# dangeross/rust-bitcoinconsensus

Measured on AMD Instinct MI355X. Metric: ECDSA verifies/sec (node) at 1/2/4/8 MI355X; % of int-ALU roofline, higher is better.
Workload: dtype u32; 1 GPU; C2: synthetic P2WPKH inputs, BIP143 sighash + ECDSA verify (BASELINE.json configs[1]); inputs_per_gpu=1000000, global_inputs=1000000, parallelism=shard x1 (independent tuples, no collective)

## Files before the change

### rust-bitcoinconsensus_amd/csrc/pipeline.h

```cpp
#pragma once
#include <cstddef>
#include <cstdint>
#include <algorithm>
#include <cstring>
#include <vector>
#include <functional>

namespace bcc {

void* pinned_alloc(size_t bytes);
void pinned_free(void* p, size_t bytes) noexcept;
void pinned_trim();
template <class T>
struct PinnedAlloc {
    using value_type = T;
    PinnedAlloc() = default;
    template <class U>
    PinnedAlloc(const PinnedAlloc<U>&) {}
    T* allocate(size_t n) { return static_cast<T*>(pinned_alloc(n * sizeof(T))); }
    void deallocate(T* p, size_t n) noexcept { pinned_free(p, n * sizeof(T)); }
    template <class U>
    bool operator==(const PinnedAlloc<U>&) const { return true; }
    template <class U>
    bool operator!=(const PinnedAlloc<U>&) const { return false; }
// ... 392 lines not shown
    void pre_upload(unsigned t, const TupleRows& rows);
    int stage_der(const DerTuples& t);
    int run(void* stream, const LateMsgFill* late = nullptr);
    int run_sighash(void* stream);
    int run_ecdsa(void* stream);
    int fetch_verdicts(uint8_t* out);
    int fetch_msgs(uint8_t* out);
    size_t n_tuples() const { return n_rows_; }
    size_t n_key_hashes() const { return n_hash_; }
    size_t n_pre() const { return n_pre_ + n_tjob_ + n_wjob_; }
    size_t n_wtx() const { return n_wtx_; }
    size_t sighash_bytes() const { return sighash_bytes_; }
    size_t n_aux() const { return n_aux_; }
    size_t pre_blocks() const { return pre_blocks_ + tjob_blocks_; }
    size_t aux_blocks() const { return aux_blocks_; }
    int device() const { return dev_; }
    uint8_t *d_tag = nullptr, *d_x = nullptr, *d_y = nullptr, *d_r = nullptr, *d_s = nullptr,
            *d_m = nullptr, *d_v = nullptr;

private:
    int sync();
    void* pick(void* stream);
    int launch_front(struct ihipStream_t* st);
    int upload_on(struct ihipStream_t* rows_stream, struct ihipStream_t* rest_stream, int part = 3);
    bool up_pending_ = false;
    struct UpCopy {
        size_t dst;
        const void* src;
        size_t len;
        bool rows;
    };
    std::vector<UpCopy> up_copies_;
    bool up_msg_one_ = false;
    static constexpr unsigned PRE_MAX_SHARDS = 64;
    std::vector<uint8_t*> pre_buf_;
    size_t pre_cap_ = 0;
    std::vector<size_t> pre_rows_;
    unsigned pre_P_ = 0;
    bool pre_armed_ = false;
    void* pre_stream_ = nullptr;
    void* ev_pre_ = nullptr;
    bool gather_pending_ = false;
    std::vector<size_t> gather_row0_;
    int launch_after_front(struct ihipStream_t* st);
    int launch_key_hash(struct ihipStream_t* st);
    int run_stages(void* stream, const LateMsgFill* late);
    int put_late(struct ihipStream_t* st, const LateMsgFill* late);
    std::vector<uint32_t> late_rows_;
    std::vector<uint8_t> late_digs_;
    void* late_host_ = nullptr;
    uint8_t* late_dev_ = nullptr;
    size_t late_cap_ = 0;
    bool kh_done_ = false;
    int dev_;
    void* own_stream_ = nullptr;
    void* last_stream_ = nullptr;
    void* side_stream_ = nullptr;
    void* ev_fork_ = nullptr;
    void* ev_join_ = nullptr;
    void* ev_up_ = nullptr;
    void* ev_rows_up_ = nullptr;
    void* ev_block_ = nullptr;
    int wait(void* stream);
    SigScratch scratch_;
    void* arena_ = nullptr;
    size_t cap_ = 0;
    void* host_image_ = nullptr;
    size_t host_cap_ = 0;
    void* vbuf_ = nullptr;
    size_t vcap_ = 0;
    void* vbuf_dev_ = nullptr;
    bool v_queued_ = false;
    int ensure_vbuf();
    int queue_verdicts(struct ihipStream_t* st);
    size_t n_rows_ = 0, n_pre_ = 0, n_aux_ = 0, n_patch_ = 0, pre_blocks_ = 0, aux_blocks_ = 0;
    uint8_t *d_aux_ = nullptr, *d_pre_ = nullptr, *d_auxd_ = nullptr;
    uint32_t *d_aux_off_ = nullptr, *d_aux_nblk_ = nullptr, *d_pre_off_ = nullptr,
             *d_pre_nblk_ = nullptr, *d_pre_row_ = nullptr;
    PatchRec* d_patch_ = nullptr;
    size_t n_tjob_ = 0, tjob_blocks_ = 0;
    uint8_t *d_tpl_ = nullptr, *d_code_ = nullptr;
    TplJob* d_tjob_ = nullptr;
    size_t n_wtx_ = 0, n_wjob_ = 0, n_win_ = 0, sighash_bytes_ = 0;
    uint8_t *d_txraw_ = nullptr, *d_txd_ = nullptr, *d_zeros_ = nullptr;
    WtxRec* d_wtx_ = nullptr;
    WinJob* d_wjob_ = nullptr;
    uint32_t* d_intab_ = nullptr;
    size_t n_hash_ = 0;
    uint32_t* d_hrow_ = nullptr;
    uint8_t* d_hprog_ = nullptr;
    uint32_t* d_emap_ = nullptr;
    uint32_t* d_mmap_ = nullptr;
    size_t n_der_ = 0;
    const uint8_t *d_pub_ = nullptr, *d_sig_ = nullptr;
    const uint64_t *d_pub_off_ = nullptr, *d_sig_off_ = nullptr;
    uint64_t pub_base_ = 0, pub_bytes_ = 0, sig_base_ = 0, sig_bytes_ = 0;

public:
    int early_launch(const TupleRows* const* rows, size_t P, const SighashJobs* const* jobs = nullptr);
    void early_reset();
    size_t early_rows() const { return early_n_; }

private:
    void* early_stream_ = nullptr;
    void* ev_early_ = nullptr;
    bool early_pending_ = false;
    size_t early_n_ = 0;
    SigScratch early_scratch_;
    void* early_arena_ = nullptr;
    size_t early_cap_ = 0;
    void* early_host_ = nullptr;
    size_t early_host_cap_ = 0;
    void* early_sig_stream_ = nullptr;
    void* ev_early_up_ = nullptr;
    void* ev_early_sig_ = nullptr;
    bool early_msgs_ = false;
    uint8_t* early_msg_ = nullptr;
};

int gpu_early_launch(int device, const TupleRows* const* rows, size_t P,
                     const SighashJobs* const* jobs = nullptr);
void gpu_early_reset(int device);

void set_stage_threads(unsigned n);

void set_direct_upload(bool on);
bool direct_upload();

void release_device_thread_state();
void release_tuple_thread_state();

int tuple_thread_buffers(int device, size_t dbytes, size_t hbytes, void** dbuf, void** hbuf,
                         void** stream);
int comb_device_tables(int* dev, const uint32_t** gcomb, int* cus);

int gpu_verify_batch(int device, const SighashJobs& jobs, const TupleRows& rows, uint8_t* verdict,
                     double* stage_seconds = nullptr);
struct StagedRound;
StagedRound* gpu_staged_new(int device);
void gpu_staged_free(StagedRound* s);
int gpu_staged_stage(StagedRound* s, const SighashJobs* const* jobs, const TupleRows* const* rows,
                     size_t parts, double* stage_seconds);
int gpu_staged_pre_arm(StagedRound* s, unsigned P, size_t cap_rows);
void gpu_staged_pre_upload(StagedRound* s, unsigned t, const TupleRows& rows);
int gpu_staged_stage_der(StagedRound* s, const DerTuples& t, double* stage_seconds);
int gpu_verify_der(int device, const DerTuples& t, uint8_t* verdict);
int gpu_staged_run(StagedRound* s, uint8_t* verdict, const LateMsgFill* late);
int gpu_staged_launch(StagedRound* s, const LateMsgFill* late);
int gpu_staged_finish(StagedRound* s, uint8_t* verdict);

int gpu_verify_parts(int device, const SighashJobs* const* jobs, const TupleRows* const* rows,
                     size_t parts, uint8_t* verdict, double* stage_seconds = nullptr,
                     const LateMsgFill* late = nullptr);

}
```

### rust-bitcoinconsensus_amd/csrc/sighash.hip

```cpp
#include <atomic>
#include <chrono>
#include <cstdlib>
#include <memory>
#include <mutex>
#include <new>
#include <thread>
#include <vector>
#include <cstring>
#include <cstdio>

#include "gpu_common.h"
#include "pipeline.h"
#include "sha256_device.h"
#include "host/hashes.h"
#include "host/team.h"

namespace bcc {

__device__ __forceinline__ uint32_t bswap_u32(uint32_t x) { return __builtin_bswap32(x); }

struct ShaMid {
    uint32_t s[8];
};

template <bool kDouble, bool kMid>
__device__ __forceinline__ void sha256_msg_lane(const uint8_t* __restrict__ buf,
                                                const uint32_t* __restrict__ off_blk,
                                                const uint32_t* __restrict__ nblk, uint32_t m,
                                                uint8_t* __restrict__ out,
                                                const uint32_t* __restrict__ out_row,
                                                const ShaMid& mid) {
    const uint4* p = reinterpret_cast<const uint4*>(buf + (size_t)off_blk[m] * 64);
    uint32_t st[8];
    if (kMid) {
#pragma unroll
        for (int k = 0; k < 8; k++) st[k] = mid.s[k];
    } else {
        sha256_init_state(st);
    }
    const uint32_t nb = nblk[m];
    uint4 nxt[4];
#pragma unroll
    for (int q = 0; q < 4; q++) nxt[q] = p[q];
    for (uint32_t b = 0; b < nb; b++) {
        uint32_t w[16];
#pragma unroll
        for (int q = 0; q < 4; q++) {
            w[4 * q + 0] = bswap_u32(nxt[q].x);
            w[4 * q + 1] = bswap_u32(nxt[q].y);
            w[4 * q + 2] = bswap_u32(nxt[q].z);
            w[4 * q + 3] = bswap_u32(nxt[q].w);
        }
        if (b + 1 < nb) {
#pragma unroll
            for (int q = 0; q < 4; q++) nxt[q] = p[(b + 1) * 4 + q];
        }
        sha256_compress(st, w);
    }
    uint32_t d[8];
    if (kDouble) {
        sha256_of_digest(d, st);
    } else {
#pragma unroll
        for (int k = 0; k < 8; k++) d[k] = st[k];
    }
    uint32_t row = out_row ? out_row[m] : m;
    uint4* o = reinterpret_cast<uint4*>(out + (size_t)row * 32);
    o[0] = make_uint4(bswap_u32(d[0]), bswap_u32(d[1]), bswap_u32(d[2]), bswap_u32(d[3]));
    o[1] = make_uint4(bswap_u32(d[4]), bswap_u32(d[5]), bswap_u32(d[6]), bswap_u32(d[7]));
}

__device__ __forceinline__ void sha256d_msg_lane(const uint8_t* __restrict__ buf,
                                                 const uint32_t* __restrict__ off_blk,
                                                 const uint32_t* __restrict__ nblk, uint32_t m,
                                                 uint8_t* __restrict__ out,
                                                 const uint32_t* __restrict__ out_row) {
    sha256_msg_lane<true, false>(buf, off_blk, nblk, m, out, out_row, ShaMid{});
}

__global__ __launch_bounds__(256) void sha256d_msgs_kernel(const uint8_t* __restrict__ buf,
                                                           const uint32_t* __restrict__ off_blk,
                                                           const uint32_t* __restrict__ nblk,
                                                           uint32_t nmsg, uint8_t* __restrict__ out,
                                                           const uint32_t* __restrict__ out_row) {
    uint32_t m = blockIdx.x * blockDim.x + threadIdx.x;
    if (m < nmsg) sha256d_msg_lane(buf, off_blk, nblk, m, out, out_row);
}

__global__ __launch_bounds__(64) void sha256_aux_kernel(const uint8_t* __restrict__ buf,
                                                        const uint32_t* __restrict__ off_blk,
                                                        const uint32_t* __restrict__ nblk,
                                                        uint32_t n, uint8_t* __restrict__ out) {
    uint32_t m = blockIdx.x * blockDim.x + threadIdx.x;
    if (m < n) sha256_msg_lane<false, false>(buf, off_blk, nblk, m, out, nullptr, ShaMid{});
}

// ... 124 lines not shown
        tpl_words(g, 64 * b, nxt, w);
        if (b + 1 < fast_blocks) tpl_fetch(m, g, 64 * (b + 1), nxt);
        sha256_compress(st, w);
    }
    const uint32_t nblk = tpl_nblk(j);
    for (uint32_t b = fast_blocks; b < nblk; b++) {
        uint32_t w[16];
#pragma unroll
        for (int k = 0; k < 16; k++) w[k] = tpl_word(m, 64 * b + 4 * k);
        sha256_compress(st, w);
    }
    uint32_t d[8];
    sha256_of_digest(d, st);
    uint4* o = reinterpret_cast<uint4*>(out + (size_t)j.row * 32);
    o[0] = make_uint4(bswap_u32(d[0]), bswap_u32(d[1]), bswap_u32(d[2]), bswap_u32(d[3]));
    o[1] = make_uint4(bswap_u32(d[4]), bswap_u32(d[5]), bswap_u32(d[6]), bswap_u32(d[7]));
}

constexpr int XS_SLOT = 100;
constexpr int XS_WG = 64;

__device__ __noinline__ void xs_compress(uint8_t* slot) {
    const uint32_t* b = reinterpret_cast<const uint32_t*>(slot);
    uint32_t* st = reinterpret_cast<uint32_t*>(slot + 64);
    uint32_t w[16], s8[8];
#pragma unroll
    for (int k = 0; k < 16; k++) w[k] = bswap_u32(b[k]);
#pragma unroll
    for (int k = 0; k < 8; k++) s8[k] = st[k];
    sha256_compress(s8, w);
#pragma unroll
    for (int k = 0; k < 8; k++) st[k] = s8[k];
}

struct XSha {
    uint8_t* slot;
    uint32_t fill;
    uint32_t total;
};

__device__ __forceinline__ void xs_init(XSha& h, uint8_t* slot) {
    h.slot = slot;
    h.fill = 0;
    h.total = 0;
    uint32_t* st = reinterpret_cast<uint32_t*>(slot + 64);
    uint32_t iv[8];
    sha256_init_state(iv);
#pragma unroll
    for (int k = 0; k < 8; k++) st[k] = iv[k];
}

__device__ __forceinline__ void xs_put(XSha& h, const uint8_t* __restrict__ src, uint32_t n) {
    h.total += n;
    while (n) {
        const uint32_t take = min(n, 64u - h.fill);
        const uintptr_t a = reinterpret_cast<uintptr_t>(src);
        const uint32_t* w = reinterpret_cast<const uint32_t*>(a & ~(uintptr_t)3);
        const uint32_t sh = (uint32_t)(a & 3), nd = (sh + take + 3) >> 2;
        uint32_t v[17];
#pragma unroll
        for (int k = 0; k < 17; k++) v[k] = (uint32_t)k < nd ? w[k] : 0u;
        uint32_t r[16];
#pragma unroll
        for (int k = 0; k < 16; k++) r[k] = __builtin_amdgcn_alignbyte(v[k + 1], v[k], sh);
        uint8_t* dst = h.slot + h.fill;
        if ((h.fill & 3) == 0) {
            uint32_t* d4 = reinterpret_cast<uint32_t*>(dst);
#pragma unroll
            for (int k = 0; k < 16; k++)
                if ((uint32_t)(4 * k) < take) d4[k] = r[k];
        } else {
#pragma unroll
            for (int i = 0; i < 64; i++)
                if ((uint32_t)i < take) dst[i] = (uint8_t)(r[i >> 2] >> (8 * (i & 3)));
        }
        h.fill += take;
        src += take;
        n -= take;
        if (h.fill == 64) {
            xs_compress(h.slot);
            h.fill = 0;
        }
    }
}

__device__ __forceinline__ void xs_final_d(XSha& h, uint8_t* __restrict__ out) {
    const uint64_t bits = (uint64_t)h.total * 8;
    h.slot[h.fill++] = 0x80;
    if (h.fill > 56) {
        while (h.fill < 64) h.slot[h.fill++] = 0;
        xs_compress(h.slot);
        h.fill = 0;
    }
    while (h.fill < 56) h.slot[h.fill++] = 0;
#pragma unroll
    for (int k = 0; k < 8; k++) h.slot[56 + k] = (uint8_t)(bits >> (8 * (7 - k)));
    xs_compress(h.slot);
    const uint32_t* st = reinterpret_cast<const uint32_t*>(h.slot + 64);
    uint32_t d[8], e[8];
#pragma unroll
    for (int k = 0; k < 8; k++) d[k] = st[k];
    sha256_of_digest(e, d);
    uint4* o = reinterpret_cast<uint4*>(out);
    o[0] = make_uint4(bswap_u32(e[0]), bswap_u32(e[1]), bswap_u32(e[2]), bswap_u32(e[3]));
    o[1] = make_uint4(bswap_u32(e[4]), bswap_u32(e[5]), bswap_u32(e[6]), bswap_u32(e[7]));
}

constexpr int XW_BYTES = 128;
struct XWin {
    uint8_t* w;
    const uint32_t* t4;
    uint32_t base;
    uint32_t nd;
};

__device__ __noinline__ void xw_refill(uint8_t* w, const uint32_t* __restrict__ t4, uint32_t nd,
                                       uint32_t base) {
    const uint32_t d0 = base >> 2;
    uint32_t v[XW_BYTES / 4];
#pragma unroll
    for (int k = 0; k < XW_BYTES / 4; k++) v[k] = d0 + k < nd ? t4[d0 + k] : 0u;
    uint32_t* w4 = reinterpret_cast<uint32_t*>(w);
#pragma unroll
    for (int k = 0; k < XW_BYTES / 4; k++) w4[k] = v[k];
}

__device__ __forceinline__ uint32_t xw_byte(XWin& x, uint32_t pos) {
    if (pos - x.base >= (uint32_t)XW_BYTES) {
        x.base = pos & ~3u;
        xw_refill(x.w, x.t4, x.nd, x.base);
    }
    return x.w[pos - x.base];
}

__device__ __forceinline__ uint32_t wire_cs(XWin& x, uint32_t& pos) {
    const uint32_t c = xw_byte(x, pos++);
    if (c < 253) return c;
    uint32_t v = xw_byte(x, pos) | xw_byte(x, pos + 1) << 8;
    if (c == 253) {
        pos += 2;
        return v;
    }
    v |= xw_byte(x, pos + 2) << 16 | xw_byte(x, pos + 3) << 24;
    pos += c == 254 ? 4 : 8;
    return v;
}

__device__ __forceinline__ uint32_t be_word_at(const uint32_t* __restrict__ t4, uint32_t off) {
    const uint32_t q = off >> 2;
    return bswap_u32(__builtin_amdgcn_alignbyte(t4[q + 1], t4[q], off & 3));
}

template <class W>
__device__ __forceinline__ void sha256d_words(W word, uint32_t L, uint8_t* __restrict__ out) {
    uint32_t st[8];
    sha256_init_state(st);
    const uint32_t nb = (L + 8) / 64 + 1, full = L >> 2, rem = L & 3;
    for (uint32_t b = 0; b < nb; b++) {
        uint32_t w[16];
#pragma unroll
        for (int q = 0; q < 16; q++) {
            const uint32_t m = 16 * b + q;
            uint32_t v;
            if (m < full) {
                v = word(m);
            } else if (m == full) {
                const uint32_t d = rem ? word(m) : 0u;
                const uint32_t keep = rem ? 0xFFFFFFFFu << (32 - 8 * rem) : 0u;
                v = (d & keep) | (0x80u << (24 - 8 * rem));
            } else {
                v = 0u;
            }
            if (b + 1 == nb && q == 14) v = (uint32_t)((uint64_t)L >> 29);
            if (b + 1 == nb && q == 15) v = L << 3;
            w[q] = v;
        }
        sha256_compress(st, w);
    }
    uint32_t d[8];
    sha256_of_digest(d, st);
    uint4* o = reinterpret_cast<uint4*>(out);
    o[0] = make_uint4(bswap_u32(d[0]), bswap_u32(d[1]), bswap_u32(d[2]), bswap_u32(d[3]));
    o[1] = make_uint4(bswap_u32(d[4]), bswap_u32(d[5]), bswap_u32(d[6]), bswap_u32(d[7]));
}

__device__ __forceinline__ uint32_t wire_input(XWin& x, uint32_t& pos, uint32_t* seq) {
    const uint32_t po = pos;
    pos += 36;
// ... 45 lines not shown
                p0 = p1;
                p1 = p2;
                p2 = next();
                kf++;
            }
            uint32_t w[16];
#pragma unroll
            for (int q = 0; q < 16; q++) {
                const uint32_t m = 16 * b + q, k = m / 9;
                uint32_t v = 0u;
                if (m < L / 4) {
                    const uint32_t kk = k - kf;
                    const uint32_t po = kk == 0 ? p0 : kk == 1 ? p1 : p2;
                    v = be_word_at(t4, po + 4 * (m - 9 * k));
                } else if (m == L / 4) {
                    v = 0x80000000u;
                }
                if (b + 1 == nb && q == 14) v = L >> 29;
                if (b + 1 == nb && q == 15) v = L << 3;
                w[q] = v;
            }
            sha256_compress(st, w);
        }
        while (np < nin) next();
    } else if (role == 1) {
        const uint32_t L = 4 * nin, nb = (L + 8) / 64 + 1;
        for (uint32_t b = 0; b < nb; b++) {
            uint32_t w[16];
#pragma unroll
            for (int q = 0; q < 16; q++) {
                const uint32_t m = 16 * b + q;
                uint32_t v = 0u;
                if (m < nin) {
                    uint32_t sq;
                    wire_input(x, pos, &sq);
                    v = be_word_at(t4, sq);
                } else if (m == nin) {
                    v = 0x80000000u;
                }
                if (b + 1 == nb && q == 14) v = L >> 29;
                if (b + 1 == nb && q == 15) v = L << 3;
                w[q] = v;
            }
            sha256_compress(st, w);
        }
    } else {
        for (uint32_t k = 0; k < nin; k++) {
            uint32_t sq;
            wire_input(x, pos, &sq);
        }
        const uint32_t nout = wire_cs(x, pos), o0 = pos;
        for (uint32_t k = 0; k < nout && pos < r.tx_len; k++) {
            pos += 8;
            pos += wire_cs(x, pos);
        }
        const uint32_t o1 = min(pos, r.tx_len);
        sha256d_words([&](uint32_t m) { return be_word_at(t4, o0 + 4 * m); }, o1 - o0, d + 64);
        return;
    }
    uint32_t dd[8];
    sha256_of_digest(dd, st);
    uint4* o = reinterpret_cast<uint4*>(d + 32 * role);
    o[0] = make_uint4(bswap_u32(dd[0]), bswap_u32(dd[1]), bswap_u32(dd[2]), bswap_u32(dd[3]));
    o[1] = make_uint4(bswap_u32(dd[4]), bswap_u32(dd[5]), bswap_u32(dd[6]), bswap_u32(dd[7]));
}

__global__ __launch_bounds__(XS_WG) void sighash_front_kernel(
    const uint8_t* __restrict__ txraw, const WtxRec* __restrict__ recs, uint32_t nwtx,
    uint32_t* __restrict__ intab, uint8_t* __restrict__ txd, const uint8_t* __restrict__ tpl,
    const uint8_t* __restrict__ code, const TplJob* __restrict__ tjobs, uint32_t ntpl,
    const uint8_t* __restrict__ aux, const uint32_t* __restrict__ aux_off,
    const uint32_t* __restrict__ aux_nblk, uint32_t naux, uint8_t* __restrict__ auxd,
    uint8_t* __restrict__ msg) {
    __shared__ __attribute__((aligned(16))) uint8_t lds[XS_WG * (XW_BYTES + 4)];
    const uint32_t g = blockIdx.x * blockDim.x + threadIdx.x, nw = 3 * nwtx;
    if (g < nw)
        bip143_tx_lane(txraw, recs, nwtx, g, intab, txd, lds + threadIdx.x * (XW_BYTES + 4));
    else if (g - nw < ntpl)
        sha256d_tpl_lane(tpl, code, tjobs, g - nw, msg);
    else if (g - nw - ntpl < naux)
        sha256d_msg_lane(aux, aux_off, aux_nblk, g - nw - ntpl, auxd, nullptr);
}

__global__ __launch_bounds__(XS_WG) void bip143_in_kernel(const uint8_t* __restrict__ txraw,
                                                          const WtxRec* __restrict__ recs,
                                                          const WinJob* __restrict__ jobs,
                                                          uint32_t n, const uint32_t* __restrict__ intab,
                                                          const uint8_t* __restrict__ txd,
                                                          const uint8_t* __restrict__ code,
                                                          const uint8_t* __restrict__ zeros,
                                                          uint8_t* __restrict__ msg) {
    __shared__ __attribute__((aligned(16))) uint8_t lds[XS_WG * XS_SLOT];
    const uint32_t i = blockIdx.x * blockDim.x + threadIdx.x;
    if (i >= n) return;
    const WinJob* jp = jobs + i;
    const WinJob j = *jp;
    const WtxRec r = recs[j.tx];
    const uint8_t* t = txraw + r.tx_off;
    const uint8_t* d = txd + 96 * (size_t)j.tx;
    const uint32_t* tab = intab + 2 * ((size_t)r.in_base + j.nin);
    const bool acp = (j.hashtype & 0x80) != 0, none = (j.hashtype & 0x1f) == 2;
    XSha h;
    xs_init(h, lds + threadIdx.x * XS_SLOT);
    xs_put(h, t, 4);
    xs_put(h, acp ? zeros : d, 32);
    xs_put(h, acp || none ? zeros : d + 32, 32);
    xs_put(h, t + tab[0], 36);
    xs_put(h, code + j.code_off, j.code_len);
    xs_put(h, reinterpret_cast<const uint8_t*>(&jp->amount_lo), 8);
    xs_put(h, t + tab[1], 4);
    xs_put(h, none ? zeros : d + 64, 32);
    xs_put(h, t + r.tx_len - 4, 4);
    xs_put(h, reinterpret_cast<const uint8_t*>(&jp->hashtype), 4);
    xs_final_d(h, msg + 32 * (size_t)j.row);
}


__device__ __forceinline__ void xs_final_s(XSha& h, uint8_t* __restrict__ out) {
    const uint64_t bits = (uint64_t)h.total * 8;
    h.slot[h.fill++] = 0x80;
    if (h.fill > 56) {
        while (h.fill < 64) h.slot[h.fill++] = 0;
        xs_compress(h.slot);
        h.fill = 0;
    }
    while (h.fill < 56) h.slot[h.fill++] = 0;
#pragma unroll
    for (int k = 0; k < 8; k++) h.slot[56 + k] = (uint8_t)(bits >> (8 * (7 - k)));
    xs_compress(h.slot);
    const uint32_t* st = reinterpret_cast<const uint32_t*>(h.slot + 64);
    uint32_t* o = reinterpret_cast<uint32_t*>(out);
#pragma unroll
    for (int k = 0; k < 8; k++) o[k] = bswap_u32(st[k]);
}

__device__ __forceinline__ void xs_put_le(XSha& h, uint32_t v, uint32_t n) {
    h.total += n;
    for (uint32_t k = 0; k < n; k++) {
        h.slot[h.fill++] = (uint8_t)(v >> (8 * k));
        if (h.fill == 64) {
            xs_compress(h.slot);
            h.fill = 0;
        }
    }
}

__device__ __forceinline__ uint32_t wire_txout(XWin& x, uint32_t& pos) {
    const uint32_t p0 = pos;
    pos += 8;
    pos += wire_cs(x, pos);
    return pos - p0;
}

__global__ __launch_bounds__(XS_WG) void taproot_tx_kernel(const uint8_t* __restrict__ raw,
                                                           const TtxRec* __restrict__ recs,
                                                           uint32_t n, uint32_t* __restrict__ intab,
                                                           uint8_t* __restrict__ ttxd) {
    __shared__ __attribute__((aligned(16))) uint8_t lds[XS_WG * (XW_BYTES + 4 + XS_SLOT)];
    const uint32_t g = blockIdx.x * blockDim.x + threadIdx.x;
    if (g >= 5 * n) return;
    const uint32_t role = g / n, i = g - role * n;
    const TtxRec r = recs[i];
    const bool spent_side = role == 1 || role == 2;
    const uint8_t* t = raw + (spent_side ? r.sp_off : r.tx_off);
    const uint32_t len = spent_side ? r.sp_len : r.tx_len;
    uint8_t* slot = lds + threadIdx.x * (XW_BYTES + 4 + XS_SLOT);
    XWin x;
    x.w = slot + XS_SLOT;
    x.t4 = reinterpret_cast<const uint32_t*>(t);
    x.nd = (len + 3) >> 2;
    x.base = 0;
    xw_refill(x.w, x.t4, x.nd, 0);
    XSha h;
    xs_init(h, slot);
    uint32_t* tab = intab + 4 * (size_t)r.in_base;
    uint32_t pos = 0;
    if (spent_side) {
        const uint32_t cnt = min(wire_cs(x, pos), r.n_in);
        for (uint32_t k = 0; k < cnt; k++) {
            const uint32_t p0 = pos, l = wire_txout(x, pos);
            if (role == 1) {
                tab[4 * k + 2] = p0;
                tab[4 * k + 3] = l;
                xs_put(h, t + p0, 8);
            } else {
                xs_put(h, t + p0 + 8, l - 8);
            }
        }
    } else {
        pos = 4;
        uint32_t nin = wire_cs(x, pos);
        if (nin == 0 && xw_byte(x, pos++) != 0) nin = wire_cs(x, pos);
        nin = min(nin, r.n_in);
        if (role == 4) {
            for (uint32_t k = 0; k < nin; k++) {
                uint32_t sq;
                wire_input(x, pos, &sq);
// ... 332 lines not shown
    std::lock_guard<std::mutex> g(pp.mu);
    pp.pageable.push_back(q);
    return q;
}
void pinned_free(void* q, size_t bytes) noexcept {
    if (!q) return;
    PinPool& pp = pin_pool();
    std::lock_guard<std::mutex> g(pp.mu);
    try {
        pp.free_[pin_class(bytes ? bytes : 1)].push_back(q);
    } catch (...) {
    }
}
void pinned_trim() {
    PinPool& pp = pin_pool();
    std::lock_guard<std::mutex> g(pp.mu);
    for (auto& l : pp.free_) {
        for (void* q : l) {
            auto it = std::find(pp.pageable.begin(), pp.pageable.end(), q);
            if (it != pp.pageable.end()) {
                pp.pageable.erase(it);
                free(q);
            } else {
                (void)hipHostFree(q);
            }
        }
        l.clear();
        l.shrink_to_fit();
    }
}

static size_t align256(size_t x) { return (x + 255) & ~(size_t)255; }

int DeviceBatch::stage(const SighashJobs& j, const TupleRows& rows) {
    const SighashJobs* jp = &j;
    const TupleRows* rp = &rows;
    return stage_parts(&jp, &rp, 1);
}

int DeviceBatch::stage_parts(const SighashJobs* const* J, const TupleRows* const* Rw, size_t P,
                             bool direct_arg) {
    if (int e = sync()) return e;
    n_der_ = 0;
    std::vector<size_t> row0(P + 1, 0), auxb0(P + 1, 0), preb0(P + 1, 0), auxi0(P + 1, 0),
        prei0(P + 1, 0), pat0(P + 1, 0), tpl0(P + 1, 0), code0(P + 1, 0), tj0(P + 1, 0),
        raw0(P + 1, 0), wtx0(P + 1, 0), wj0(P + 1, 0), win0(P + 1, 0), h0(P + 1, 0);
    for (size_t p = 0; p < P; p++) {
        row0[p + 1] = row0[p] + Rw[p]->size();
        auxb0[p + 1] = auxb0[p] + J[p]->aux.size();
        preb0[p + 1] = preb0[p] + J[p]->pre.size();
        auxi0[p + 1] = auxi0[p] + J[p]->aux_off.size();
        prei0[p + 1] = prei0[p] + J[p]->pre_off.size();
        pat0[p + 1] = pat0[p] + J[p]->patches.size();
        tpl0[p + 1] = tpl0[p] + J[p]->tpl.size();
        code0[p + 1] = code0[p] + J[p]->code.size();
        tj0[p + 1] = tj0[p] + J[p]->tjobs.size();
        raw0[p + 1] = raw0[p] + J[p]->txraw.size();
        wtx0[p + 1] = wtx0[p] + J[p]->wtx.size();
        wj0[p + 1] = wj0[p] + J[p]->wjobs.size();
        win0[p + 1] = win0[p] + J[p]->win_entries;
        h0[p + 1] = h0[p] + Rw[p]->hrow.size();
    }
    std::vector<size_t> part_tjblk(P, 0), part_wbytes(P, 0);
    const size_t LIM = (size_t)1 << 32;
    if (auxb0[P] >= LIM || preb0[P] >= LIM || tpl0[P] >= LIM || code0[P] >= LIM ||
        raw0[P] >= LIM || row0[P] >= LIM || win0[P] >= LIM / 2) {
        fprintf(stderr, "[bcc] DeviceBatch::stage_parts: a job blob exceeds 4 GiB; split the round\n");
        return (int)hipErrorInvalidValue;
    }
    n_rows_ = row0[P];
    n_pre_ = prei0[P];
    n_aux_ = auxi0[P];
    n_patch_ = pat0[P];
    pre_blocks_ = preb0[P] / 64;
    aux_blocks_ = auxb0[P] / 64;
    n_tjob_ = tj0[P];

    n_wtx_ = wtx0[P];
    n_wjob_ = wj0[P];
    n_win_ = win0[P];
    n_hash_ = h0[P];
    const size_t R = n_rows_;
    enum { TAG, X, RR, S, EMAP, MMAP, AUX, PRE, AUX_OFF, AUX_NBLK, PRE_OFF, PRE_NBLK, PRE_ROW, PATCH,
           TPL, CODE, TJOB, TXRAW, WTX, WJOB, HROW, HPROG, ZEROS, UPLOADED, Y = UPLOADED, M, V, AUXD, INTAB, TXD,
           NB };
    bool need_y = false, need_m = false, need_e = false, need_mm = false;
    for (size_t p = 0; p < P; p++) {
        need_y |= !Rw[p]->y_unused && Rw[p]->size() != 0;
        need_m |= !Rw[p]->msg_one && Rw[p]->size() != 0;
        need_e |= !Rw[p]->emap.empty();
        need_mm |= !Rw[p]->mmap.empty();
    }
    need_e = need_e && early_n_ != 0;
    need_mm = need_mm && early_n_ != 0 && early_msgs_;
    size_t sizes[NB] = {};
    sizes[TAG] = R; sizes[X] = sizes[Y] = sizes[RR] = sizes[S] = sizes[M] = 32 * R;
    sizes[EMAP] = need_e ? 4 * R : 0;
    sizes[MMAP] = need_mm ? 4 * R : 0;
    sizes[AUX] = auxb0[P]; sizes[PRE] = preb0[P];
    sizes[AUX_OFF] = sizes[AUX_NBLK] = 4 * n_aux_;
    sizes[PRE_OFF] = sizes[PRE_NBLK] = sizes[PRE_ROW] = 4 * n_pre_;
    sizes[PATCH] = sizeof(PatchRec) * n_patch_;
    sizes[TPL] = tpl0[P]; sizes[CODE] = code0[P]; sizes[TJOB] = sizeof(TplJob) * n_tjob_;
    sizes[TXRAW] = raw0[P]; sizes[WTX] = sizeof(WtxRec) * n_wtx_; sizes[WJOB] = sizeof(WinJob) * n_wjob_;
    sizes[HROW] = 4 * n_hash_; sizes[HPROG] = 20 * n_hash_;
    sizes[ZEROS] = 64;
    sizes[V] = R; sizes[AUXD] = 32 * n_aux_; sizes[INTAB] = 8 * n_win_; sizes[TXD] = 96 * n_wtx_;
    size_t off[NB], total = 0;
    for (int i = 0; i < NB; i++) {
        off[i] = total;
        total += align256(sizes[i]);
    }
    const size_t upload = off[UPLOADED], upload_ym = off[V];
    if (total > cap_) {
        if (arena_) BCC_HIP_TRY(hipFree(arena_));
        arena_ = nullptr;
        cap_ = 0;
        BCC_HIP_TRY(hipMalloc(&arena_, total));
        cap_ = total;
    }
    if (upload_ym > host_cap_) {
        if (host_image_) BCC_HIP_TRY(hipHostFree(host_image_));
        host_image_ = nullptr;
        host_cap_ = 0;
        BCC_HIP_TRY(hipHostMalloc(&host_image_, upload_ym, hipHostMallocDefault));
        host_cap_ = upload_ym;
    }
    uint8_t* a = (uint8_t*)arena_;
    d_tag = a + off[TAG]; d_x = a + off[X]; d_y = a + off[Y]; d_r = a + off[RR]; d_s = a + off[S];
    d_m = a + off[M]; d_v = a + off[V]; d_aux_ = a + off[AUX]; d_pre_ = a + off[PRE];
    d_auxd_ = a + off[AUXD];
    d_aux_off_ = (uint32_t*)(a + off[AUX_OFF]); d_aux_nblk_ = (uint32_t*)(a + off[AUX_NBLK]);
    d_pre_off_ = (uint32_t*)(a + off[PRE_OFF]); d_pre_nblk_ = (uint32_t*)(a + off[PRE_NBLK]);
    d_pre_row_ = (uint32_t*)(a + off[PRE_ROW]); d_patch_ = (PatchRec*)(a + off[PATCH]);
    d_tpl_ = a + off[TPL]; d_code_ = a + off[CODE]; d_tjob_ = (TplJob*)(a + off[TJOB]);
    d_txraw_ = a + off[TXRAW]; d_wtx_ = (WtxRec*)(a + off[WTX]); d_wjob_ = (WinJob*)(a + off[WJOB]);
    d_hrow_ = (uint32_t*)(a + off[HROW]); d_hprog_ = a + off[HPROG];
    d_zeros_ = a + off[ZEROS]; d_intab_ = (uint32_t*)(a + off[INTAB]); d_txd_ = a + off[TXD];
    d_emap_ = need_e ? (uint32_t*)(a + off[EMAP]) : nullptr;
    d_mmap_ = need_mm ? (uint32_t*)(a + off[MMAP]) : nullptr;
    uint8_t* h = (uint8_t*)host_image_;
    memset(h + off[ZEROS], 0, 64);
    constexpr size_t DIRECT_MIN_PIECE = (size_t)256 << 10, DIRECT_MIN_ROWS = 65536;
    bool dm[NB] = {};
    if (direct_arg && direct_upload() && P && R >= DIRECT_MIN_ROWS) {
        for (int b : {TAG, X, RR, S, AUX, PRE, TPL, CODE, TXRAW, HPROG})
            dm[b] = sizes[b] / P >= DIRECT_MIN_PIECE;
    }
    bool gathered = direct_arg && pre_armed_ && pre_P_ == P && R < ((size_t)1 << 32);
    for (size_t p = 0; gathered && p < P; p++) gathered = pre_rows_[p] == Rw[p]->size();
    pre_armed_ = false;
    gather_pending_ = gathered;
    if (gathered) {
        gather_row0_.assign(row0.begin(), row0.end());
        for (int b : {TAG, X, RR, S}) dm[b] = true;
    }
    auto fill_rows = [&](size_t p, size_t lo, size_t hi) {
        const TupleRows& rw = *Rw[p];
        const size_t r0 = row0[p] + lo, nr = hi - lo;
        auto cp = [&](int b, size_t at, const void* src, size_t len) {
            if (len) memcpy(h + off[b] + at, src, len);
        };
        if (!dm[TAG]) cp(TAG, r0, rw.tag.data() + lo, nr);
        if (!dm[X]) cp(X, 32 * r0, rw.x.data() + 32 * lo, 32 * nr);
        if (!dm[RR]) cp(RR, 32 * r0, rw.r.data() + 32 * lo, 32 * nr);
        if (!dm[S]) cp(S, 32 * r0, rw.s.data() + 32 * lo, 32 * nr);
        if (need_y && nr) rw.copy_y(h + off[Y] + 32 * r0, lo, hi);
        if (need_m && nr) rw.copy_msg(h + off[M] + 32 * r0, lo, hi);
        if (need_e && nr) rw.copy_emap((uint32_t*)(h + off[EMAP]) + r0, lo, hi);
        if (need_mm && nr) rw.copy_mmap((uint32_t*)(h + off[MMAP]) + r0, lo, hi);
    };
    auto fill = [&](size_t p) {
        const SighashJobs& j = *J[p];
        const TupleRows& rw = *Rw[p];
        const size_t r0 = row0[p];
        auto cp = [&](int b, size_t at, const void* src, size_t len) {
            if (len) memcpy(h + off[b] + at, src, len);
        };
        if (!dm[AUX]) cp(AUX, auxb0[p], j.aux.data(), j.aux.size());
        if (!dm[PRE]) cp(PRE, preb0[p], j.pre.data(), j.pre.size());
        if (!dm[TPL]) cp(TPL, tpl0[p], j.tpl.data(), j.tpl.size());
        if (!dm[CODE]) cp(CODE, code0[p], j.code.data(), j.code.size());
        if (!dm[TXRAW]) cp(TXRAW, raw0[p], j.txraw.data(), j.txraw.size());
        if (!dm[HPROG]) cp(HPROG, 20 * h0[p], rw.hprog.data(), rw.hprog.size());
        const uint32_t ablk = (uint32_t)(auxb0[p] / 64), pblk = (uint32_t)(preb0[p] / 64);
        uint32_t* ao = (uint32_t*)(h + off[AUX_OFF]) + auxi0[p];
        for (size_t k = 0; k < j.aux_off.size(); k++) ao[k] = j.aux_off[k] + ablk;
        cp(AUX_NBLK, 4 * auxi0[p], j.aux_nblk.data(), 4 * j.aux_nblk.size());
        uint32_t* po = (uint32_t*)(h + off[PRE_OFF]) + prei0[p];
        uint32_t* pr = (uint32_t*)(h + off[PRE_ROW]) + prei0[p];
        for (size_t k = 0; k < j.pre_off.size(); k++) {
            po[k] = j.pre_off[k] + pblk;
            pr[k] = j.pre_row[k] + (uint32_t)r0;
        }
        cp(PRE_NBLK, 4 * prei0[p], j.pre_nblk.data(), 4 * j.pre_nblk.size());
        PatchRec* pt = (PatchRec*)(h + off[PATCH]) + pat0[p];
        for (size_t k = 0; k < j.patches.size(); k++)
            pt[k] = PatchRec{j.patches[k].pre_byte + pblk * 64, j.patches[k].aux + (uint32_t)auxi0[p]};
        TplJob* tj = (TplJob*)(h + off[TJOB]) + tj0[p];
        size_t wb = 0, tb = 0;
        for (size_t k = 0; k < j.tjobs.size(); k++) {
            TplJob t = j.tjobs[k];
            tb += tpl_job_blocks(t);
            t.tpl_off += (uint32_t)tpl0[p];
            t.code_off += (uint32_t)code0[p];
            t.row += (uint32_t)r0;
            if (!need_mm) t.nblk &= ~TPL_EARLY;
            tj[k] = t;
        }
        WtxRec* wr = (WtxRec*)(h + off[WTX]) + wtx0[p];
        for (size_t k = 0; k < j.wtx.size(); k++) {
            WtxRec t = j.wtx[k];
            wb += t.tx_len + 96;
            t.tx_off += (uint32_t)raw0[p];
            t.in_base += (uint32_t)win0[p];
            wr[k] = t;
        }
        WinJob* wj = (WinJob*)(h + off[WJOB]) + wj0[p];
        for (size_t k = 0; k < j.wjobs.size(); k++) {
            WinJob t = j.wjobs[k];
            wb += t.code_len + sizeof(WinJob) + 32;
            t.tx += (uint32_t)wtx0[p];
            t.code_off += (uint32_t)code0[p];
            t.row += (uint32_t)r0;
            wj[k] = t;
// ... 228 lines not shown
    while (hi - lo > 1) {
        const uint32_t mid = (lo + hi) / 2;
        if (g.row0[mid] <= row) lo = mid;
        else hi = mid;
    }
    const size_t k = row - g.row0[lo];
    const uint8_t* b = g.base[lo];
    tag[row] = b[k];
    const uint4* xs = reinterpret_cast<const uint4*>(b + g.xoff) + 2 * k;
    const uint4* rs = reinterpret_cast<const uint4*>(b + g.xoff + 32 * (size_t)g.cap) + 2 * k;
    const uint4* ss = reinterpret_cast<const uint4*>(b + g.xoff + 64 * (size_t)g.cap) + 2 * k;
    x[2 * row] = xs[0];
    x[2 * row + 1] = xs[1];
    r[2 * row] = rs[0];
    r[2 * row + 1] = rs[1];
    s[2 * row] = ss[0];
    s[2 * row + 1] = ss[1];
}

__global__ void __launch_bounds__(256) msg_one_kernel(uint4* __restrict__ m, size_t n) {
    const size_t k = (size_t)blockIdx.x * blockDim.x + threadIdx.x;
    if (k >= n) return;
    m[2 * k] = make_uint4(1u, 0u, 0u, 0u);
    m[2 * k + 1] = make_uint4(0u, 0u, 0u, 0u);
}

int DeviceBatch::upload_on(hipStream_t rows_stream, hipStream_t rest_stream, int part) {
    if (!up_pending_) return 0;
    uint8_t* a = (uint8_t*)arena_;
    if (part & 1) {
        if (gather_pending_) {
            gather_pending_ = false;
            BCC_HIP_TRY(hipEventRecord((hipEvent_t)ev_pre_, (hipStream_t)pre_stream_));
            BCC_HIP_TRY(hipStreamWaitEvent(rows_stream, (hipEvent_t)ev_pre_, 0));
            RowGather g{};
            g.P = pre_P_;
            g.xoff = (uint32_t)pre_x_off(pre_cap_);
            g.cap = (uint32_t)pre_cap_;
            for (unsigned p = 0; p < pre_P_; p++) {
                g.base[p] = pre_buf_[p];
                g.row0[p] = (uint32_t)gather_row0_[p];
            }
            g.row0[pre_P_] = (uint32_t)gather_row0_[pre_P_];
            if (n_rows_) {
                hipLaunchKernelGGL(row_gather_kernel, dim3((unsigned)((n_rows_ + 255) / 256)), dim3(256), 0,
                                   rows_stream, g, (uint8_t*)d_tag, (uint4*)d_x, (uint4*)d_r, (uint4*)d_s,
                                   (uint32_t)n_rows_);
                BCC_HIP_TRY(hipGetLastError());
            }
        }
        for (const UpCopy& c : up_copies_)
            if (c.rows || !rest_stream)
                BCC_HIP_TRY(hipMemcpyAsync(a + c.dst, c.src, c.len, hipMemcpyHostToDevice, rows_stream));
        if (rest_stream) {
            if (!ev_rows_up_) {
                hipEvent_t e = nullptr;
                BCC_HIP_TRY(hipEventCreateWithFlags(&e, hipEventDisableTiming));
                ev_rows_up_ = e;
            }
            BCC_HIP_TRY(hipEventRecord((hipEvent_t)ev_rows_up_, rows_stream));
        }
    }
    if (part & 2) {
        up_pending_ = false;
        if (rest_stream) {
            BCC_HIP_TRY(hipStreamWaitEvent(rest_stream, (hipEvent_t)ev_rows_up_, 0));
            for (const UpCopy& c : up_copies_)
                if (!c.rows)
                    BCC_HIP_TRY(hipMemcpyAsync(a + c.dst, c.src, c.len, hipMemcpyHostToDevice, rest_stream));
        }
        if (up_msg_one_) {
            up_msg_one_ = false;
            hipStream_t ms = rest_stream ? rest_stream : rows_stream;
            hipLaunchKernelGGL(msg_one_kernel, dim3((unsigned)((n_rows_ + 255) / 256)), dim3(256), 0, ms,
                               (uint4*)d_m, n_rows_);
            BCC_HIP_TRY(hipGetLastError());
        }
    }
    return 0;
}

int DeviceBatch::launch_after_front(hipStream_t st) {
    if (n_wjob_) {
        hipLaunchKernelGGL(bip143_in_kernel, dim3((unsigned)((n_wjob_ + XS_WG - 1) / XS_WG)),
                           dim3(XS_WG), 0, st, d_txraw_, d_wtx_, d_wjob_, (uint32_t)n_wjob_,
                           d_intab_, d_txd_, d_code_, d_zeros_, d_m);
        BCC_HIP_TRY(hipGetLastError());
    }
    if (n_patch_) {
        size_t th = n_patch_;
        hipLaunchKernelGGL(patch_digests_kernel, dim3((unsigned)((th + 255) / 256)), dim3(256), 0, st,
                           d_pre_, d_patch_, d_auxd_, (uint32_t)n_patch_);
        BCC_HIP_TRY(hipGetLastError());
    }
    if (n_pre_) {
        hipLaunchKernelGGL(sha256d_msgs_kernel, dim3((unsigned)((n_pre_ + 255) / 256)), dim3(256), 0, st,
                           d_pre_, d_pre_off_, d_pre_nblk_, (uint32_t)n_pre_, d_m, d_pre_row_);
        BCC_HIP_TRY(hipGetLastError());
    }
    return 0;
}

int DeviceBatch::launch_front(hipStream_t st) {
    const size_t lanes = 3 * n_wtx_ + n_tjob_ + n_aux_;
    if (lanes) {
        hipLaunchKernelGGL(sighash_front_kernel, dim3((unsigned)((lanes + XS_WG - 1) / XS_WG)),
                           dim3(XS_WG), 0, st, d_txraw_, d_wtx_, (uint32_t)n_wtx_, d_intab_, d_txd_,
                           d_tpl_, d_code_, d_tjob_, (uint32_t)n_tjob_, d_aux_, d_aux_off_,
                           d_aux_nblk_, (uint32_t)n_aux_, d_auxd_, d_m);
        BCC_HIP_TRY(hipGetLastError());
    }
    return launch_after_front(st);
}

int DeviceBatch::run_sighash(void* stream) {
    BCC_HIP_TRY(hipSetDevice(dev_));
    hipStream_t st = (hipStream_t)pick(stream);
    if (!st) return (int)hipErrorOutOfMemory;
    if (int e = upload_on(st, nullptr)) return e;
    return launch_front(st);
}

int DeviceBatch::run_ecdsa(void* stream) {
    BCC_HIP_TRY(hipSetDevice(dev_));
    void* st = pick(stream);
    if (!st) return (int)hipErrorOutOfMemory;
    if (int e = upload_on((hipStream_t)st, nullptr)) return e;
    if (n_der_)
        if (int e = der_launch(d_pub_, d_pub_off_, pub_base_, pub_bytes_, d_sig_, d_sig_off_, sig_base_,
                               sig_bytes_, n_der_, d_tag, d_x, d_y, d_r, d_s, st))
            return e;
    if (int e = ecdsa_launch(scratch_, d_tag, d_x, d_y, d_r, d_s, d_m, d_v, n_rows_, st)) return e;
    return launch_key_hash((hipStream_t)st);
}

__global__ void __launch_bounds__(256) key_hash_kernel(const uint8_t* __restrict__ tag,
                                                       const uint8_t* __restrict__ x,
                                                       const uint8_t* __restrict__ y,
                                                       const uint32_t* __restrict__ hrow,
                                                       const uint8_t* __restrict__ hprog,
                                                       uint32_t n, uint8_t* __restrict__ verdict) {
    const uint32_t k = blockIdx.x * blockDim.x + threadIdx.x;
    if (k >= n) return;
    const uint32_t row = hrow[k];
    const uint32_t t = tag[row];
    uint32_t xw[8], yw[8], d[5];
    const uint4* xp = (const uint4*)(x + 32 * (size_t)row);
    const uint4 x0 = xp[0], x1 = xp[1];
    xw[0] = sha_bswap(x0.x); xw[1] = sha_bswap(x0.y); xw[2] = sha_bswap(x0.z); xw[3] = sha_bswap(x0.w);
    xw[4] = sha_bswap(x1.x); xw[5] = sha_bswap(x1.y); xw[6] = sha_bswap(x1.z); xw[7] = sha_bswap(x1.w);
    if (t == 2 || t == 3) {
#pragma unroll
        for (int i = 0; i < 8; i++) yw[i] = 0;
    } else {
        const uint4* yp = (const uint4*)(y + 32 * (size_t)row);
        const uint4 y0 = yp[0], y1 = yp[1];
        yw[0] = sha_bswap(y0.x); yw[1] = sha_bswap(y0.y); yw[2] = sha_bswap(y0.z); yw[3] = sha_bswap(y0.w);
        yw[4] = sha_bswap(y1.x); yw[5] = sha_bswap(y1.y); yw[6] = sha_bswap(y1.z); yw[7] = sha_bswap(y1.w);
    }
    key_hash160(t, xw, yw, d);
    const uint8_t* pg = hprog + 20 * (size_t)k;
    uint32_t diff = 0;
#pragma unroll
    for (int i = 0; i < 20; i++) diff |= (uint32_t)pg[i] ^ ((d[i / 4] >> (8 * (i % 4))) & 0xffu);
    if (diff) verdict[row] = 0;
}

int DeviceBatch::launch_key_hash(hipStream_t st) {
    if (!n_hash_) return 0;
// ... 618 lines not shown
```

Baseline: 117.0 million verifies/s.

## Assemble BIP143 sighash words directly in registers instead of byte-streaming through LDS

Replaces the byte-wise streaming SHA state (xs_put/xs_final_d with a per-lane LDS slot and a zeros buffer) in the per-input BIP143 kernel with a word-level construction. Each message word is computed from aligned dword loads using alignbyte/alignbit, and only a small 15-word tail row is kept in LDS. The kernel is templated on workgroup size and launched with 256 threads when there is enough work. This is meant to remove byte-granular loops, branches and LDS traffic in sighash preimage assembly, at the cost of more intricate offset and padding logic that must be correct for every script-code length and alignment.

After: 118.0 million verifies/s, median of 6. About the same (+0.8%).

```diff
diff --git a/rust-bitcoinconsensus_amd/csrc/pipeline.h b/rust-bitcoinconsensus_amd/csrc/pipeline.h
--- a/rust-bitcoinconsensus_amd/csrc/pipeline.h
+++ b/rust-bitcoinconsensus_amd/csrc/pipeline.h
@@ -498,7 +498,7 @@
     uint8_t *d_tpl_ = nullptr, *d_code_ = nullptr;
     TplJob* d_tjob_ = nullptr;
     size_t n_wtx_ = 0, n_wjob_ = 0, n_win_ = 0, sighash_bytes_ = 0;
-    uint8_t *d_txraw_ = nullptr, *d_txd_ = nullptr, *d_zeros_ = nullptr;
+    uint8_t *d_txraw_ = nullptr, *d_txd_ = nullptr;
     WtxRec* d_wtx_ = nullptr;
     WinJob* d_wjob_ = nullptr;
     uint32_t* d_intab_ = nullptr;
diff --git a/rust-bitcoinconsensus_amd/csrc/sighash.hip b/rust-bitcoinconsensus_amd/csrc/sighash.hip
--- a/rust-bitcoinconsensus_amd/csrc/sighash.hip
+++ b/rust-bitcoinconsensus_amd/csrc/sighash.hip
@@ -12,6 +12,7 @@
 #include "gpu_common.h"
 #include "pipeline.h"
 #include "sha256_device.h"
+#include "win_words.h"
 #include "host/hashes.h"
 #include "host/team.h"
 
@@ -302,28 +303,6 @@
             h.fill = 0;
         }
     }
-}
-
-__device__ __forceinline__ void xs_final_d(XSha& h, uint8_t* __restrict__ out) {
-    const uint64_t bits = (uint64_t)h.total * 8;
-    h.slot[h.fill++] = 0x80;
-    if (h.fill > 56) {
-        while (h.fill < 64) h.slot[h.fill++] = 0;
-        xs_compress(h.slot);
-        h.fill = 0;
-    }
-    while (h.fill < 56) h.slot[h.fill++] = 0;
-#pragma unroll
-    for (int k = 0; k < 8; k++) h.slot[56 + k] = (uint8_t)(bits >> (8 * (7 - k)));
-    xs_compress(h.slot);
-    const uint32_t* st = reinterpret_cast<const uint32_t*>(h.slot + 64);
-    uint32_t d[8], e[8];
-#pragma unroll
-    for (int k = 0; k < 8; k++) d[k] = st[k];
-    sha256_of_digest(e, d);
-    uint4* o = reinterpret_cast<uint4*>(out);
-    o[0] = make_uint4(bswap_u32(e[0]), bswap_u32(e[1]), bswap_u32(e[2]), bswap_u32(e[3]));
-    o[1] = make_uint4(bswap_u32(e[4]), bswap_u32(e[5]), bswap_u32(e[6]), bswap_u32(e[7]));
 }
 
 constexpr int XW_BYTES = 128;
@@ -535,37 +514,38 @@
         sha256d_msg_lane(aux, aux_off, aux_nblk, g - nw - ntpl, auxd, nullptr);
 }
 
-__global__ __launch_bounds__(XS_WG) void bip143_in_kernel(const uint8_t* __restrict__ txraw,
-                                                          const WtxRec* __restrict__ recs,
-                                                          const WinJob* __restrict__ jobs,
-                                                          uint32_t n, const uint32_t* __restrict__ intab,
-                                                          const uint8_t* __restrict__ txd,
-                                                          const uint8_t* __restrict__ code,
-                                                          const uint8_t* __restrict__ zeros,
-                                                          uint8_t* __restrict__ msg) {
-    __shared__ __attribute__((aligned(16))) uint8_t lds[XS_WG * XS_SLOT];
+constexpr int WIN_WG = 256;
+template <int kWG>
+__global__ __launch_bounds__(kWG) void bip143_in_kernel(const uint8_t* __restrict__ txraw,
+                                                        const WtxRec* __restrict__ recs,
+                                                        const WinJob* __restrict__ jobs,
+                                                        uint32_t n, const uint32_t* __restrict__ intab,
+                                                        const uint8_t* __restrict__ txd,
+                                                        const uint8_t* __restrict__ code,
+                                                        uint8_t* __restrict__ msg) {
+    __shared__ uint32_t lds[kWG * WIN_ROW];
     const uint32_t i = blockIdx.x * blockDim.x + threadIdx.x;
     if (i >= n) return;
-    const WinJob* jp = jobs + i;
-    const WinJob j = *jp;
+    const WinJob j = jobs[i];
     const WtxRec r = recs[j.tx];
-    const uint8_t* t = txraw + r.tx_off;
-    const uint8_t* d = txd + 96 * (size_t)j.tx;
-    const uint32_t* tab = intab + 2 * ((size_t)r.in_base + j.nin);
-    const bool acp = (j.hashtype & 0x80) != 0, none = (j.hashtype & 0x1f) == 2;
-    XSha h;
-    xs_init(h, lds + threadIdx.x * XS_SLOT);
-    xs_put(h, t, 4);
-    xs_put(h, acp ? zeros : d, 32);
-    xs_put(h, acp || none ? zeros : d + 32, 32);
-    xs_put(h, t + tab[0], 36);
-    xs_put(h, code + j.code_off, j.code_len);
-    xs_put(h, reinterpret_cast<const uint8_t*>(&jp->amount_lo), 8);
-    xs_put(h, t + tab[1], 4);
-    xs_put(h, none ? zeros : d + 64, 32);
-    xs_put(h, t + r.tx_len - 4, 4);
-    xs_put(h, reinterpret_cast<const uint8_t*>(&jp->hashtype), 4);
-    xs_final_d(h, msg + 32 * (size_t)j.row);
+    const uint2 tab = *reinterpret_cast<const uint2*>(intab + 2 * ((size_t)r.in_base + j.nin));
+    WinSrc s;
+    s.t4 = reinterpret_cast<const uint32_t*>(txraw + r.tx_off);
+    s.d4 = reinterpret_cast<const uint32_t*>(txd + 96 * (size_t)j.tx);
+    s.c4 = reinterpret_cast<const uint32_t*>(code);
+    s.tx_len = r.tx_len;
+    s.outpoint = tab.x;
+    s.seq = tab.y;
+    s.code_off = j.code_off;
+    s.code_len = j.code_len;
+    s.hashtype = j.hashtype;
+    s.amount_lo = j.amount_lo;
+    s.amount_hi = j.amount_hi;
+    uint32_t d[8];
+    win_sighash_lane(s, lds + threadIdx.x * WIN_ROW, d);
+    uint4* o = reinterpret_cast<uint4*>(msg + 32 * (size_t)j.row);
+    o[0] = make_uint4(bswap_u32(d[0]), bswap_u32(d[1]), bswap_u32(d[2]), bswap_u32(d[3]));
+    o[1] = make_uint4(bswap_u32(d[4]), bswap_u32(d[5]), bswap_u32(d[6]), bswap_u32(d[7]));
 }
 
 
@@ -1064,7 +1044,7 @@
     n_hash_ = h0[P];
     const size_t R = n_rows_;
     enum { TAG, X, RR, S, EMAP, MMAP, AUX, PRE, AUX_OFF, AUX_NBLK, PRE_OFF, PRE_NBLK, PRE_ROW, PATCH,
-           TPL, CODE, TJOB, TXRAW, WTX, WJOB, HROW, HPROG, ZEROS, UPLOADED, Y = UPLOADED, M, V, AUXD, INTAB, TXD,
+           TPL, CODE, TJOB, TXRAW, WTX, WJOB, HROW, HPROG, UPLOADED, Y = UPLOADED, M, V, AUXD, INTAB, TXD,
            NB };
     bool need_y = false, need_m = false, need_e = false, need_mm = false;
     for (size_t p = 0; p < P; p++) {
@@ -1086,7 +1066,6 @@
     sizes[TPL] = tpl0[P]; sizes[CODE] = code0[P]; sizes[TJOB] = sizeof(TplJob) * n_tjob_;
     sizes[TXRAW] = raw0[P]; sizes[WTX] = sizeof(WtxRec) * n_wtx_; sizes[WJOB] = sizeof(WinJob) * n_wjob_;
     sizes[HROW] = 4 * n_hash_; sizes[HPROG] = 20 * n_hash_;
-    sizes[ZEROS] = 64;
     sizes[V] = R; sizes[AUXD] = 32 * n_aux_; sizes[INTAB] = 8 * n_win_; sizes[TXD] = 96 * n_wtx_;
     size_t off[NB], total = 0;
     for (int i = 0; i < NB; i++) {
@@ -1118,11 +1097,10 @@
     d_tpl_ = a + off[TPL]; d_code_ = a + off[CODE]; d_tjob_ = (TplJob*)(a + off[TJOB]);
     d_txraw_ = a + off[TXRAW]; d_wtx_ = (WtxRec*)(a + off[WTX]); d_wjob_ = (WinJob*)(a + off[WJOB]);
     d_hrow_ = (uint32_t*)(a + off[HROW]); d_hprog_ = a + off[HPROG];
-    d_zeros_ = a + off[ZEROS]; d_intab_ = (uint32_t*)(a + off[INTAB]); d_txd_ = a + off[TXD];
+    d_intab_ = (uint32_t*)(a + off[INTAB]); d_txd_ = a + off[TXD];
     d_emap_ = need_e ? (uint32_t*)(a + off[EMAP]) : nullptr;
     d_mmap_ = need_mm ? (uint32_t*)(a + off[MMAP]) : nullptr;
     uint8_t* h = (uint8_t*)host_image_;
-    memset(h + off[ZEROS], 0, 64);
     constexpr size_t DIRECT_MIN_PIECE = (size_t)256 << 10, DIRECT_MIN_ROWS = 65536;
     bool dm[NB] = {};
     if (direct_arg && direct_upload() && P && R >= DIRECT_MIN_ROWS) {
@@ -1517,9 +1495,14 @@
 
 int DeviceBatch::launch_after_front(hipStream_t st) {
     if (n_wjob_) {
-        hipLaunchKernelGGL(bip143_in_kernel, dim3((unsigned)((n_wjob_ + XS_WG - 1) / XS_WG)),
-                           dim3(XS_WG), 0, st, d_txraw_, d_wtx_, d_wjob_, (uint32_t)n_wjob_,
-                           d_intab_, d_txd_, d_code_, d_zeros_, d_m);
+        if (n_wjob_ >= WIN_WG)
+            hipLaunchKernelGGL(bip143_in_kernel<WIN_WG>, dim3((unsigned)((n_wjob_ + WIN_WG - 1) / WIN_WG)),
+                               dim3(WIN_WG), 0, st, d_txraw_, d_wtx_, d_wjob_, (uint32_t)n_wjob_,
+                               d_intab_, d_txd_, d_code_, d_m);
+        else
+            hipLaunchKernelGGL(bip143_in_kernel<XS_WG>, dim3((unsigned)((n_wjob_ + XS_WG - 1) / XS_WG)),
+                               dim3(XS_WG), 0, st, d_txraw_, d_wtx_, d_wjob_, (uint32_t)n_wjob_,
+                               d_intab_, d_txd_, d_code_, d_m);
         BCC_HIP_TRY(hipGetLastError());
     }
     if (n_patch_) {
diff --git a/rust-bitcoinconsensus_amd/csrc/win_words.h b/rust-bitcoinconsensus_amd/csrc/win_words.h
--- /dev/null
+++ b/rust-bitcoinconsensus_amd/csrc/win_words.h
@@ -0,0 +1,152 @@
+#pragma once
+#include <stdint.h>
+
+#include "sha256_device.h"
+
+#ifndef BCC_HD
+#if defined(__HIPCC__)
+#define BCC_HD __host__ __device__ __attribute__((always_inline)) inline
+#else
+#define BCC_HD inline
+#endif
+#endif
+
+namespace bcc {
+
+constexpr int WIN_ROW = 15;
+constexpr int WIN_HEAD = 26;
+
+struct WinSrc {
+    const uint32_t* t4;
+    const uint32_t* d4;
+    const uint32_t* c4;
+    uint32_t tx_len;
+    uint32_t outpoint, seq;
+    uint32_t code_off, code_len;
+    uint32_t hashtype;
+    uint32_t amount_lo, amount_hi;
+};
+
+BCC_HD uint32_t win_min(uint32_t a, uint32_t b) { return a < b ? a : b; }
+
+BCC_HD uint32_t win_bswap(uint32_t x) { return __builtin_bswap32(x); }
+
+BCC_HD uint32_t win_alignbyte(uint32_t hi, uint32_t lo, uint32_t sh) {
+#if defined(__HIP_DEVICE_COMPILE__)
+    return __builtin_amdgcn_alignbyte(hi, lo, sh);
+#else
+    return sh ? (lo >> (8 * sh)) | (hi << (32 - 8 * sh)) : lo;
+#endif
+}
+
+BCC_HD uint32_t win_alignbit(uint32_t hi, uint32_t lo, uint32_t sh) {
+#if defined(__HIP_DEVICE_COMPILE__)
+    return __builtin_amdgcn_alignbit(hi, lo, sh);
+#else
+    return sh ? (lo >> sh) | (hi << (32 - sh)) : lo;
+#endif
+}
+
+template <int kN>
+BCC_HD void win_load(const uint32_t* p, uint32_t* v) {
+    __builtin_memcpy(v, p, 4 * kN);
+}
+
+BCC_HD uint32_t win_be_word(const uint32_t* a4, uint32_t off, uint32_t last) {
+    const uint32_t q = off >> 2;
+    return win_bswap(win_alignbyte(a4[win_min(q + 1, last)], a4[win_min(q, last)], off & 3));
+}
+
+BCC_HD uint32_t win_code_dword(const WinSrc& s, uint32_t idx) {
+    const uint32_t first = s.code_off >> 2, last = (s.code_off + s.code_len - 1) >> 2;
+    return idx - first <= last - first ? s.c4[idx] : 0u;
+}
+
+BCC_HD void win_head_words(const WinSrc& s, uint32_t (&w)[WIN_HEAD]) {
+    const bool acp = (s.hashtype & 0x80) != 0, none = (s.hashtype & 0x1f) == 2;
+    uint32_t d[16], o[12];
+#pragma unroll
+    for (int k = 0; k < 4; k++) win_load<4>(s.d4 + 4 * k, d + 4 * k);
+    const uint32_t q = s.outpoint >> 2, sh = s.outpoint & 3;
+    win_load<4>(s.t4 + q, o);
+    win_load<4>(s.t4 + q + 4, o + 4);
+    win_load<2>(s.t4 + q + 8, o + 8);
+    w[0] = win_bswap(s.t4[0]);
+#pragma unroll
+    for (int k = 0; k < 8; k++) w[1 + k] = acp ? 0u : win_bswap(d[k]);
+#pragma unroll
+    for (int k = 0; k < 8; k++) w[9 + k] = acp || none ? 0u : win_bswap(d[8 + k]);
+#pragma unroll
+    for (int k = 0; k < 9; k++) w[17 + k] = win_bswap(win_alignbyte(o[k + 1], o[k], sh));
+}
+
+BCC_HD void win_tail_row(const WinSrc& s, uint32_t* row) {
+    const bool none = (s.hashtype & 0x1f) == 2;
+    const uint32_t tlast = (s.tx_len - 1) >> 2, cr = s.code_len & 3;
+    const uint32_t mq = (s.code_off >> 2) + (s.code_len >> 2);
+    const uint32_t meet =
+        win_bswap(win_alignbyte(win_code_dword(s, mq + 1), win_code_dword(s, mq), s.code_off & 3));
+    uint32_t ho[8];
+    win_load<4>(s.d4 + 16, ho);
+    win_load<4>(s.d4 + 20, ho + 4);
+    row[0] = meet >> ((32 - 8 * cr) & 31);
+    row[1] = win_bswap(s.amount_lo);
+    row[2] = win_bswap(s.amount_hi);
+    row[3] = win_be_word(s.t4, s.seq, tlast);
+#pragma unroll
+    for (int k = 0; k < 8; k++) row[4 + k] = none ? 0u : win_bswap(ho[k]);
+    row[12] = win_be_word(s.t4, s.tx_len - 4, tlast);
+    row[13] = win_bswap(s.hashtype);
+    row[14] = 0u;
+}
+
+BCC_HD uint32_t win_tail_word(const WinSrc& s, const uint32_t* row, uint32_t k) {
+    const int32_t j = (int32_t)(k - (s.code_len >> 2));
+    const uint32_t jj = j < 0 ? 0u : j > 13 ? 13u : (uint32_t)j;
+    return win_alignbit(row[jj], row[jj + 1], 8 * (s.code_len & 3));
+}
+
+BCC_HD uint32_t win_word(const WinSrc& s, const uint32_t* row, uint32_t m) {
+    if (m < WIN_HEAD) {
+        uint32_t w[WIN_HEAD];
+        win_head_words(s, w);
+        return w[m];
+    }
+    const uint32_t k = m - WIN_HEAD, q = (s.code_off >> 2) + k;
+    if (k < s.code_len >> 2)
+        return win_bswap(win_alignbyte(win_code_dword(s, q + 1), win_code_dword(s, q), s.code_off & 3));
+    return win_tail_word(s, row, k);
+}
+
+BCC_HD void win_sighash_lane(const WinSrc& s, uint32_t* row, uint32_t (&out)[8]) {
+    const uint32_t L = 156 + s.code_len, nb = (L + 8) / 64 + 1, full = L >> 2, rem = L & 3;
+    const uint32_t keep = rem ? 0xFFFFFFFFu << (32 - 8 * rem) : 0u, mark = 0x80000000u >> (8 * rem);
+    const uint32_t cw = s.code_len >> 2, cq = s.code_off >> 2, csh = s.code_off & 3;
+    win_tail_row(s, row);
+    uint32_t st[8], w[16], h[WIN_HEAD];
+    win_head_words(s, h);
+#pragma unroll
+    for (int q = 0; q < 16; q++) w[q] = h[q];
+    sha256_init_state(st);
+    sha256_compress(st, w);
+    for (uint32_t b = 1; b < nb; b++) {
+        const uint32_t k0 = 16 * b - WIN_HEAD;
+        uint32_t cd[17];
+#pragma unroll
+        for (int q = 0; q < 17; q++) cd[q] = win_code_dword(s, cq + k0 + q);
+#pragma unroll
+        for (int q = 0; q < 16; q++) {
+            const uint32_t m = 16 * b + q, k = k0 + q;
+            uint32_t v = k < cw ? win_bswap(win_alignbyte(cd[q + 1], cd[q], csh)) : win_tail_word(s, row, k);
+            if (q < 10) v = b == 1 ? h[16 + q] : v;
+            v = m < full ? v : m == full ? (v & keep) | mark : 0u;
+            if (b + 1 == nb && q == 14) v = (uint32_t)((uint64_t)L >> 29);
+            if (b + 1 == nb && q == 15) v = L << 3;
+            w[q] = v;
+        }
+        sha256_compress(st, w);
+    }
+    sha256_of_digest(out, st);
+}
+
+}
```
